# bikuta6/nbody-deep-sim

Measured on AMD Instinct MI355X. Metric: pair-interactions/sec, direct O(N^2) leapfrog N-body, fp32, higher is better.
Workload: dtype f32; 1 GPU; Plummer sphere, 65536 particles, direct all-pairs leapfrog step (BASELINE configs[1] shape: 65536 bodies per GPU); n_particles=65536, particles_per_gpu=65536, seed=1234, parallelism=single GPU

## Files before the change

nbody-deep-sim_amd/csrc/direct_force.hip:

```cpp
#include <hip/hip_runtime.h>
#include <string.h>
#include <stdint.h>

#include "../../include/nbd.h"
#include "direct_kernels.h"

namespace {

template <bool MASKED, int KU, bool UNI = false>
__global__ __launch_bounds__(64 * kWaves, KU == 4 ? 8 : 5) void accel_kernel(
    const f4* __restrict__ src, const SrcView sv, const f4* __restrict__ tgt,
    int n_tgt, int tgt_off, float eps2, float scale, float* __restrict__ out, int out_rows, int tile_len) {
  __shared__ f4 lds[kWaves * 2 * kChunk + kWaves * 6 * 64 / 4];
  {
    const int tz = blockIdx.z * tile_len;
    src += tz; tgt += tz; out += (size_t)tz * 3;
  }
  const int lane = threadIdx.x & 63;
  const int wave = __builtin_amdgcn_readfirstlane(threadIdx.x >> 6);
  const int t_base = blockIdx.x * kTgtPerWG;
  const int i0 = t_base + lane, i1 = t_base + 64 + lane;
  const f4 t0 = tgt[min(i0, n_tgt - 1)], t1 = tgt[min(i1, n_tgt - 1)];
  const f2 xi = {t0.x, t1.x}, yi = {t0.y, t1.y}, zi = {t0.z, t1.z};
  f2 ax = {0.f, 0.f}, ay = {0.f, 0.f}, az = {0.f, 0.f};
  f2 e2 = {eps2, eps2};
  asm volatile("" : "+v"(e2));

  const int jw = blockIdx.y * kWaves + wave;
  const int c_begin = jw * sv.cpw_q + min(jw, sv.cpw_r), c_end = c_begin + sv.cpw_q + (jw < sv.cpw_r ? 1 : 0);
  f4* stage = &lds[wave * 2 * kChunk];
  const f4* s_lane = src + lane;
  auto phys = [&](int c) { return c + (c >= sv.skip_c0 ? sv.skip_cn : 0); };
  if (c_begin < c_end)
    __builtin_amdgcn_global_load_lds(GPTR(s_lane + (size_t)phys(c_begin) * kChunk), LPTR(stage), 16, 0, 0);
  for (int c = c_begin; c < c_end; ++c) {
    const int b = (c - c_begin) & 1;
    if (c + 1 < c_end) {
      __builtin_amdgcn_global_load_lds(GPTR(s_lane + (size_t)phys(c + 1) * kChunk),
                                       LPTR(stage + (b ^ 1) * kChunk), 16, 0, 0);
      asm volatile("s_waitcnt vmcnt(1)" ::: "memory");
    } else {
      asm volatile("s_waitcnt vmcnt(0)" ::: "memory");
    }
    const f4* buf = stage + b * kChunk;
    const int pc = phys(c);
    const int j0 = pc * kChunk;
    if (MASKED || pc == sv.edge0 || pc == sv.edge1 || (UNI && pc == sv.tail)) {
#pragma unroll 4
      for (int j = 0; j < kChunk; ++j)
        interact<true, UNI>(buf[j], xi, yi, zi, e2, ax, ay, az, j0 + j, tgt_off + i0, tgt_off + i1, sv);
    } else {
#pragma unroll 1
      for (int j = 0; j < kChunk; j += KU) interact_block<KU, UNI>(buf + j, xi, yi, zi, e2, ax, ay, az);
    }
  }

  float* red = reinterpret_cast<float*>(&lds[kWaves * 2 * kChunk]);
  float* mine = red + wave * 6 * 64;
  mine[0 * 64 + lane] = ax.x; mine[1 * 64 + lane] = ax.y;
  mine[2 * 64 + lane] = ay.x; mine[3 * 64 + lane] = ay.y;
  mine[4 * 64 + lane] = az.x; mine[5 * 64 + lane] = az.y;
  __syncthreads();
  float* dst = out + ((size_t)blockIdx.y * out_rows + t_base) * 3;
  const int n_valid = min(kTgtPerWG, n_tgt - t_base) * 3;
  for (int o = threadIdx.x; o < n_valid; o += 64 * kWaves) {
    const int lt = o / 3, comp = o - lt * 3;
    const int idx = (comp * 2 + (lt >> 6)) * 64 + (lt & 63);
    float sum = red[idx];
#pragma unroll
    for (int w = 1; w < kWaves; ++w) sum += red[w * 6 * 64 + idx];
    dst[o] = __fmul_rn(scale, sum);
  }
}

constexpr int kSymTile = 1024;
constexpr int kSymChunks = kSymTile / kChunk;
constexpr int kSymSlots = 16;

__device__ __forceinline__ float rol1(float x) {
  return __int_as_float(__builtin_amdgcn_mov_dpp(__float_as_int(x), 0x134 , 0xf, 0xf, false));
}

__device__ __forceinline__ void sym_pair(const f4 p, const f2 xi, const f2 yi, const f2 zi, const f2 e2,
                                         f2& ax, f2& ay, f2& az, f2& rx, f2& ry, f2& rz) {
  const f2 dx = f2{p.x, p.x} - xi, dy = f2{p.y, p.y} - yi, dz = f2{p.z, p.z} - zi;
  f2 r2 = __builtin_elementwise_fma(dx, dx, e2);
  r2 = __builtin_elementwise_fma(dy, dy, r2);
  r2 = __builtin_elementwise_fma(dz, dz, r2);
  const f2 s = {__builtin_amdgcn_rsqf(r2.x), __builtin_amdgcn_rsqf(r2.y)};
  const f2 w = (s * s) * s;
  ax = __builtin_elementwise_fma(w, dx, ax);
  ay = __builtin_elementwise_fma(w, dy, ay);
  az = __builtin_elementwise_fma(w, dz, az);
  rx = __builtin_elementwise_fma(-w, dx, rx);
  ry = __builtin_elementwise_fma(-w, dy, ry);
  rz = __builtin_elementwise_fma(-w, dz, rz);
}

template <int SG>
__global__ __launch_bounds__(256 * SG, 2 * SG) void accel_sym_kernel(const f4* __restrict__ posm, int n, int m,
                                                                     int r0, int n_slots, float eps2,
                                                                     float* __restrict__ out) {
  constexpr int CPS = kSymChunks / SG;
  constexpr int kStageF4 = SG * 2 * 2 * kChunk;
  constexpr int kRedF = 2 * 4 * SG * 3 * 64;
  constexpr int kOwnF = SG * 4 * 12 * 64;
  constexpr int kLdsF = (kStageF4 * 4 + kRedF > kOwnF) ? kStageF4 * 4 + kRedF : kOwnF;
  __shared__ f4 lds[kLdsF / 4];
  float* const ldsf = reinterpret_cast<float*>(lds);

  const int half = m >> 1, mm = m - 1;
  const int rr = blockIdx.x / half, i = blockIdx.x - rr * half, r = r0 + rr;
  const int ta = i == 0 ? r % mm : (r + i) % mm;
  const int tb = i == 0 ? mm : (r - i + mm) % mm;
  const int slot = (r + 1) % n_slots;
  const bool init = r + 1 < n_slots;

  const int lane = threadIdx.x & 63;
  const int wave = __builtin_amdgcn_readfirstlane(threadIdx.x >> 6);
  const int tg = wave & 3, sg = wave >> 2;
  const int row0 = ta * kSymTile + tg * 256 + lane;
  const f4 q0 = posm[row0], q1 = posm[row0 + 64], q2 = posm[row0 + 128], q3 = posm[row0 + 192];
  const f2 xa = {q0.x, q1.x}, ya = {q0.y, q1.y}, za = {q0.z, q1.z};
  const f2 xb = {q2.x, q3.x}, yb = {q2.y, q3.y}, zb = {q2.z, q3.z};
  f2 axa = {0.f, 0.f}, aya = {0.f, 0.f}, aza = {0.f, 0.f}, axb = {0.f, 0.f}, ayb = {0.f, 0.f}, azb = {0.f, 0.f};
  f2 e2 = {eps2, eps2};
  asm volatile("" : "+v"(e2));

  f4* const stage = &lds[sg * 4 * kChunk];
  const int c0 = tb * kSymChunks + sg * CPS;
  const f4* const s_lane = posm + lane + (size_t)c0 * kChunk;
  auto fetch = [&](int c, int b) {
    __builtin_amdgcn_global_load_lds(GPTR(s_lane + c * kChunk), LPTR(stage + b * 2 * kChunk), 16, 0, 0);
    __builtin_amdgcn_global_load_lds(GPTR(s_lane + c * kChunk), LPTR(stage + b * 2 * kChunk + kChunk), 16, 0, 0);
  };
  if (tg == 3) {
    fetch(0, 0);
    asm volatile("s_waitcnt vmcnt(0)" ::: "memory");
  }
  __syncthreads();

  for (int c = 0; c < CPS; ++c) {
    const int b = c & 1;
    if (tg == 3 && c + 1 < CPS) fetch(c + 1, b ^ 1);
    float* const o_react = out + ((size_t)slot * n + (size_t)(c0 + c) * kChunk + lane) * 3 + tg;
    float old = 0.f;
    if (!init && tg < 3) old = *o_react;
    const f4* buf = stage + b * 2 * kChunk + lane;
    f2 rx = {0.f, 0.f}, ry = {0.f, 0.f}, rz = {0.f, 0.f};
#pragma unroll 2
    for (int k = 0; k < kChunk; ++k) {
      const f4 p = buf[k];
      sym_pair(p, xa, ya, za, e2, axa, aya, aza, rx, ry, rz);
      sym_pair(p, xb, yb, zb, e2, axb, ayb, azb, rx, ry, rz);
      rx = f2{rol1(rx.x), rol1(rx.y)};
      ry = f2{rol1(ry.x), rol1(ry.y)};
      rz = f2{rol1(rz.x), rol1(rz.y)};
    }
    float* const red = ldsf + kStageF4 * 4 + b * (4 * SG * 3 * 64);
    float* const mine = red + wave * 3 * 64;
    mine[lane] = rx.x + rx.y;
    mine[64 + lane] = ry.x + ry.y;
    mine[128 + lane] = rz.x + rz.y;
    if (tg == 3 && c + 1 < CPS) asm volatile("s_waitcnt vmcnt(0)" ::: "memory");
    __syncthreads();
    if (tg < 3) {
      const float* rs = red + (sg * 4) * 3 * 64 + tg * 64 + lane;
      const float v = ((rs[0] + rs[3 * 64]) + rs[6 * 64]) + rs[9 * 64];
      *o_react = init ? v : old + v;
    }
  }

  float* const o_own = out + ((size_t)slot * n + row0) * 3;
  const f2 own[6] = {axa, aya, aza, axb, ayb, azb};
  if (SG == 1) {
#pragma unroll
    for (int t = 0; t < 4; ++t)
#pragma unroll
      for (int comp = 0; comp < 3; ++comp) {
        const f2 v2 = own[(t >> 1) * 3 + comp];
        const float v = (t & 1) ? v2.y : v2.x;
        float* o = o_own + t * 64 * 3 + comp;
        *o = init ? v : *o + v;
      }
    return;
  }
  __syncthreads();
  float* const mo = ldsf + (sg * 4 + tg) * 12 * 64;
#pragma unroll
  for (int t = 0; t < 4; ++t)
#pragma unroll
    for (int comp = 0; comp < 3; ++comp) {
      const f2 v2 = own[(t >> 1) * 3 + comp];
      mo[(comp * 4 + t) * 64 + lane] = (t & 1) ? v2.y : v2.x;
    }
  __syncthreads();
  if (sg != 0) return;
#pragma unroll
  for (int t = 0; t < 4; ++t)
#pragma unroll
    for (int comp = 0; comp < 3; ++comp) {
      const float* src = ldsf + tg * 12 * 64 + (comp * 4 + t) * 64 + lane;
      float v = src[0];
#pragma unroll
      for (int g = 1; g < SG; ++g) v += src[g * 4 * 12 * 64];
      float* o = o_own + t * 64 * 3 + comp;
      *o = init ? v : *o + v;
    }
}

__global__ __launch_bounds__(256) void finish_kernel(const float* __restrict__ slabs, int n_slabs,
                                                     size_t slab_stride, float g, float* __restrict__ acc,
                                                     float* __restrict__ vel, float c_kick, int n3) {
  __shared__ float part[4][64];
  const int lane = threadIdx.x & 63, w = threadIdx.x >> 6;
  const int i = blockIdx.x * 64 + lane;
  float sum = 0.f;
  if (i < n3)
    for (int s = w; s < n_slabs; s += 4) sum += slabs[s * slab_stride + i];
  part[w][lane] = sum;
  __syncthreads();
  if (w != 0 || i >= n3) return;
  const float a = __fmul_rn(g, (part[0][lane] + part[1][lane]) + (part[2][lane] + part[3][lane]));
  acc[i] = a;
  if (vel) vel[i] = __fadd_rn(vel[i], __fmul_rn(c_kick, a));
}

__global__ __launch_bounds__(256) void pack_kernel(const float* __restrict__ pos,
                                                   const float* __restrict__ mass, int n, int n_pad,
                                                   f4* __restrict__ posm) {
  const int i = blockIdx.x * 256 + threadIdx.x;
  if (i >= n_pad) return;
  f4 v = {0.f, 0.f, 0.f, 0.f};
  if (i < n) v = f4{pos[3 * i], pos[3 * i + 1], pos[3 * i + 2], mass[i]};
  posm[i] = v;
}

__global__ __launch_bounds__(256) void kick_drift_kernel(float* __restrict__ pos, float* __restrict__ vel,
                                                         const float* __restrict__ acc,
                                                         const float* __restrict__ mass, int n, int n_pad,
                                                         float ck, float cd, f4* __restrict__ posm) {
  const int i = blockIdx.x * 256 + threadIdx.x;
  if (i >= n_pad) return;
  f4 pm = {0.f, 0.f, 0.f, 0.f};
  if (i < n) {
    float x[3];
#pragma unroll
    for (int k = 0; k < 3; ++k) {
      float v = vel[3 * i + k];
      if (acc) { v = __fadd_rn(v, __fmul_rn(ck, acc[3 * i + k])); vel[3 * i + k] = v; }
      x[k] = __fadd_rn(pos[3 * i + k], __fmul_rn(cd, v));
      pos[3 * i + k] = x[k];
    }
    pm = f4{x[0], x[1], x[2], mass ? mass[i] : 0.f};
  }
  if (posm) posm[i] = pm;
}

__global__ __launch_bounds__(256) void zero_f32_kernel(float* __restrict__ p, size_t n) {
  const size_t i = (size_t)blockIdx.x * 256 + threadIdx.x;
  if (i < n) p[i] = 0.f;
}

__global__ __launch_bounds__(256) void snapshot_kernel(const float* __restrict__ pos, const float* __restrict__ vel,
                                                       const float* __restrict__ acc, int n3, float* __restrict__ out) {
  const int i = blockIdx.x * 256 + threadIdx.x;
  if (i >= n3) return;
  out[i] = pos[i]; out[n3 + i] = vel[i]; out[2 * n3 + i] = acc[i];
}

__global__ __launch_bounds__(256) void axpy_kernel(float* __restrict__ y, const float* __restrict__ x,
                                                   float c, int n) {
  const int i = blockIdx.x * 256 + threadIdx.x;
  if (i < n) y[i] = __fadd_rn(y[i], __fmul_rn(c, x[i]));
}

__global__ __launch_bounds__(64 * kWaves) void energy_kernel(const f4* __restrict__ posm, int n, int n_chunks,
                                                             float soft_, int all_masked,
                                                             double* __restrict__ partial_u) {
  __shared__ f4 lds[kWaves * 2 * kChunk + 8];
  const int lane = threadIdx.x & 63;
  const int wave = __builtin_amdgcn_readfirstlane(threadIdx.x >> 6);
  const int t_base = blockIdx.x * kTgtPerWG;
  const int i0 = t_base + lane, i1 = t_base + 64 + lane;
  const f4 t0 = posm[min(i0, n - 1)], t1 = posm[min(i1, n - 1)];
  const f2 xi = {t0.x, t1.x}, yi = {t0.y, t1.y}, zi = {t0.z, t1.z};
  f2 u = {0.f, 0.f};
  f2 soft = {soft_, soft_};
  asm volatile("" : "+v"(soft));
  const int c_lo = t_base / kChunk;
  const int span = n_chunks - c_lo;
  const int parts = gridDim.y * kWaves;
  const int cpw = (span + parts - 1) / parts;
  const int jw = blockIdx.y * kWaves + wave;
  const int c_begin = min(c_lo + jw * cpw, n_chunks), c_end = min(c_begin + cpw, n_chunks);
  const int c_diag_end = (t_base + kTgtPerWG + kChunk - 1) / kChunk;
  f4* stage = &lds[wave * 2 * kChunk];
  const f4* s_lane = posm + lane;
  if (c_begin < c_end)
    __builtin_amdgcn_global_load_lds(GPTR(s_lane + (size_t)c_begin * kChunk), LPTR(stage), 16, 0, 0);
  for (int c = c_begin; c < c_end; ++c) {
    const int b = (c - c_begin) & 1;
    if (c + 1 < c_end) {
      __builtin_amdgcn_global_load_lds(GPTR(s_lane + (size_t)(c + 1) * kChunk), LPTR(stage + (b ^ 1) * kChunk), 16, 0, 0);
      asm volatile("s_waitcnt vmcnt(1)" ::: "memory");
    } else {
      asm volatile("s_waitcnt vmcnt(0)" ::: "memory");
    }
    const f4* buf = stage + b * kChunk;
    const int j0 = c * kChunk;
    if (all_masked || c < c_diag_end || c == n_chunks - 1) {
#pragma unroll 4
      for (int j = 0; j < kChunk; ++j) energy_pair<true>(buf[j], xi, yi, zi, soft, u, j0 + j, i0, i1, n);
    } else {
#pragma unroll 4
      for (int j = 0; j < kChunk; ++j) energy_pair<false>(buf[j], xi, yi, zi, soft, u, j0 + j, i0, i1, n);
    }
  }
  double acc = 0.0;
  if (i0 < n) acc += (double)t0.w * (double)u.x;
  if (i1 < n) acc += (double)t1.w * (double)u.y;
  for (int off = 32; off > 0; off >>= 1) acc += __shfl_down(acc, off);
  double* red = reinterpret_cast<double*>(&lds[kWaves * 2 * kChunk]);
  if (lane == 0) red[wave] = acc;
  __syncthreads();
  if (threadIdx.x == 0)
    partial_u[(size_t)blockIdx.y * gridDim.x + blockIdx.x] = (red[0] + red[1]) + (red[2] + red[3]);
}

__global__ __launch_bounds__(256) void kinetic_kernel(const f4* __restrict__ posm, const float* __restrict__ vel,
                                                      int n, double* __restrict__ partial_k) {
  __shared__ double red[4];
  const int i = blockIdx.x * 256 + threadIdx.x;
  double k = 0.0;
  if (i < n) {
    const float vx = vel[3 * i], vy = vel[3 * i + 1], vz = vel[3 * i + 2];
    const float v2 = __fadd_rn(__fadd_rn(__fmul_rn(vx, vx), __fmul_rn(vy, vy)), __fmul_rn(vz, vz));
    k = (double)__fmul_rn(__fmul_rn(0.5f, posm[i].w), v2);
  }
  for (int off = 32; off > 0; off >>= 1) k += __shfl_down(k, off);
  if ((threadIdx.x & 63) == 0) red[threadIdx.x >> 6] = k;
  __syncthreads();
  if (threadIdx.x == 0) partial_k[blockIdx.x] = (red[0] + red[1]) + (red[2] + red[3]);
}

__global__ __launch_bounds__(256) void energy_final_kernel(const double* __restrict__ pu, int nu,
                                                           const double* __restrict__ pk, int nk, float g,
                                                           double* __restrict__ out) {
  __shared__ double ru[4], rk[4];
  double u = 0.0, k = 0.0;
  for (int b = threadIdx.x; b < nu; b += 256) u += pu[b];
  for (int b = threadIdx.x; b < nk; b += 256) k += pk[b];
  for (int off = 32; off > 0; off >>= 1) { u += __shfl_down(u, off); k += __shfl_down(k, off); }
  if ((threadIdx.x & 63) == 0) { ru[threadIdx.x >> 6] = u; rk[threadIdx.x >> 6] = k; }
  __syncthreads();
  if (threadIdx.x == 0) {
    out[0] = -(double)g * ((ru[0] + ru[1]) + (ru[2] + ru[3]));
    out[1] = (rk[0] + rk[1]) + (rk[2] + rk[3]);
  }
}

inline int energy_slabs(int groups) {
  int s = (4096 + groups - 1) / groups;
  return s < 1 ? 1 : (s > 32 ? 32 : s);
}

struct AccelPlan { int groups, slabs, n_chunks, cpw, variant; };

constexpr int kCUs = 256;
double plan_cost(int groups, int n_chunks, int slabs) {
  static const double eff[6] = {1.0, 0.70, 0.935, 0.975, 0.99, 1.0};
  const int waves = slabs * kWaves, q = n_chunks / waves, r = n_chunks % waves;
  const int wgs = groups * slabs, per_cu = ceil_div(wgs, kCUs);
  const int heavy_per_cu = ceil_div(groups * ceil_div(r, kWaves), kCUs);
  const double chunks = (double)per_cu * q + (heavy_per_cu < per_cu ? heavy_per_cu : per_cu);
  return chunks / eff[per_cu < 5 ? per_cu : 5] * (per_cu <= 5 ? 1.03 : 1.0) + 0.25 * per_cu;
}

AccelPlan plan_chunks(int n_chunks, int n_tgt) {
  AccelPlan p;
  p.variant = 0;
  p.groups = ceil_div(n_tgt, kTgtPerWG);
  p.n_chunks = n_chunks;
  int cap = n_chunks / kWaves;
  cap = cap < 1 ? 1 : (cap > kMaxSlabs ? kMaxSlabs : cap);
  int slabs;
  const int pref = ceil_div(8192, p.groups), cap_pref = n_chunks / (16 * kWaves);
  if ((pref < cap_pref ? pref : cap_pref) * p.groups >= 10 * kCUs) {
    slabs = pref < cap_pref ? pref : cap_pref;
    const int min_slabs = ceil_div(n_chunks, kWaves * 64);
    if (slabs < min_slabs) slabs = min_slabs;
  } else {
    slabs = 1;
    double best = plan_cost(p.groups, n_chunks, 1);
    for (int s = 2; s <= cap; ++s) {
      const double c = plan_cost(p.groups, n_chunks, s);
      if (c < best * 0.999) { best = c; slabs = s; }
    }
  }
  if (slabs > kMaxSlabs) slabs = kMaxSlabs;
  if (slabs < 1) slabs = 1;
  p.slabs = slabs;
  p.cpw = ceil_div(n_chunks, p.slabs * kWaves);
  return p;
}

AccelPlan plan_accel(int n_src, int n_tgt) { return plan_chunks(ceil_div(n_src, kChunk), n_tgt); }

inline int check(hipError_t e) { return e == hipSuccess ? 0 : (int)e; }
inline int launch_status() { return check(hipGetLastError()); }

SrcView full_view(int n_src, const AccelPlan& p) {
  SrcView v;
  v.n_src = n_src; v.n_chunks = p.n_chunks; v.cpw_q = 0; v.cpw_r = 0;
  v.skip_c0 = p.n_chunks; v.skip_cn = 0; v.ex_lo = 0; v.ex_hi = 0; v.edge0 = -1; v.edge1 = -1;
  v.tail = (n_src % kChunk) ? n_src / kChunk : -1;
  return v;
}

int excluded_view(int n_src, int ex_lo, int ex_hi, SrcView* v) {
  const int phys = ceil_div(n_src, kChunk);
  int c0 = ceil_div(ex_lo, kChunk), c1 = ex_hi / kChunk;
  if (ex_hi >= n_src) c1 = phys;
  if (c1 < c0) c1 = c0;
  if (v) {
    v->n_src = n_src; v->skip_c0 = c0; v->skip_cn = c1 - c0; v->ex_lo = ex_lo; v->ex_hi = ex_hi;
    v->edge0 = (ex_lo % kChunk) ? ex_lo / kChunk : -1;
    v->edge1 = (ex_hi % kChunk && ex_hi < n_src) ? ex_hi / kChunk : -1;
    if (ex_hi <= ex_lo) { v->skip_c0 = phys; v->skip_cn = 0; v->edge0 = v->edge1 = -1; }
    v->tail = (n_src % kChunk) ? n_src / kChunk : -1;
  }
  return ex_hi <= ex_lo ? phys : phys - (c1 - c0);
}

int launch_accel(const float* posm_src, SrcView sv, const float* posm_tgt, int n_tgt, int off,
                 float eps2, float direct_scale, float* slabs_or_acc, const AccelPlan& p,
                 hipStream_t st, bool uniform = false, int out_rows = 0, int tiles = 1, int tile_len = 0) {
  dim3 grid(p.groups, p.slabs, tiles), block(64 * kWaves);
  if (out_rows <= 0) out_rows = n_tgt;
  const f4* s = reinterpret_cast<const f4*>(posm_src);
  const f4* t = reinterpret_cast<const f4*>(posm_tgt);
  sv.n_chunks = p.n_chunks;
  sv.cpw_q = p.n_chunks / (p.slabs * kWaves); sv.cpw_r = p.n_chunks % (p.slabs * kWaves);
  const bool masked = eps2 < kEps2Masked;
#define NBD_LAUNCH(M, K, U) accel_kernel<M, K, U><<<grid, block, 0, st>>>(s, sv, t, n_tgt, off, eps2, direct_scale, slabs_or_acc, out_rows, tile_len)
  if (uniform) {
    if (p.variant == 1) { if (masked) NBD_LAUNCH(true, 4, true); else NBD_LAUNCH(false, 4, true); }
    else                { if (masked) NBD_LAUNCH(true, 8, true); else NBD_LAUNCH(false, 8, true); }
  } else {
    if (p.variant == 1) { if (masked) NBD_LAUNCH(true, 4, false); else NBD_LAUNCH(false, 4, false); }
    else                { if (masked) NBD_LAUNCH(true, 8, false); else NBD_LAUNCH(false, 8, false); }
  }
#undef NBD_LAUNCH
  return launch_status();
}

bool misaligned16(const void* p) { return (reinterpret_cast<uintptr_t>(p) & 15) != 0; }

struct SymPlan { int m, core, rem, slots, total_slots; };

SymPlan plan_sym(int n) {
  SymPlan p;
  p.m = n / kSymTile;
  p.m &= ~1;
  p.core = p.m * kSymTile;
  p.rem = n - p.core;
  p.slots = p.m < kSymSlots ? p.m : kSymSlots;
  p.total_slots = p.slots + (p.rem > 0 ? 1 : 0);
  return p;
}

size_t sym_workspace_bytes(int n) {
  const SymPlan p = plan_sym(n);
  return p.m < 2 ? 0 : (size_t)p.total_slots * n * 3 * sizeof(float);
}

constexpr int kSymStepMinN = 65536;
bool sym_step(int n, float eps2) { return n >= kSymStepMinN && eps2 >= kEps2Masked; }

int launch_sym(const float* posm, int n, float eps2, float* slots, hipStream_t st, int variant = 0) {
  const SymPlan sp = plan_sym(n);
  const f4* pm = reinterpret_cast<const f4*>(posm);
  AccelPlan dp;
  dp.groups = kSymTile / kTgtPerWG; dp.slabs = 1; dp.n_chunks = kSymChunks; dp.variant = 0;
  dp.cpw = ceil_div(kSymChunks, kWaves);
  int rc = launch_accel(posm, full_view(kSymTile, dp), posm, kSymTile, 0, eps2, 1.0f, slots, dp, st, true, n, sp.m,
                        kSymTile);
  if (rc) return rc;
  const int rounds = sp.m - 1;
  for (int r0 = 0; r0 < rounds;) {
    const int r1 = r0 == 0 ? (sp.slots - 1 < rounds ? sp.slots - 1 : rounds) : (r0 + sp.slots < rounds ? r0 + sp.slots : rounds);
    const int wgs = (r1 - r0) * (sp.m / 2);
    if (variant == 1) accel_sym_kernel<2><<<wgs, 512, 0, st>>>(pm, n, sp.m, r0, sp.slots, eps2, slots);
    else accel_sym_kernel<4><<<wgs, 1024, 0, st>>>(pm, n, sp.m, r0, sp.slots, eps2, slots);
    if ((rc = launch_status())) return rc;
    r0 = r1;
  }
  if (sp.rem == 0) return 0;
  AccelPlan tp;
  tp.groups = ceil_div(sp.rem, kTgtPerWG); tp.slabs = sp.total_slots; tp.n_chunks = ceil_div(n, kChunk); tp.variant = 0;
  tp.cpw = ceil_div(tp.n_chunks, tp.slabs * kWaves);
  rc = launch_accel(posm, full_view(n, tp), posm + (size_t)sp.core * 4, sp.rem, sp.core, eps2, 1.0f,
                    slots + (size_t)sp.core * 3, tp, st, true, n);
  if (rc) return rc;
  SrcView sv;
  AccelPlan cp;
  cp.n_chunks = excluded_view(n, 0, sp.core, &sv);
  cp.groups = sp.core / kTgtPerWG; cp.slabs = 1; cp.variant = 0; cp.cpw = ceil_div(cp.n_chunks, kWaves);
  return launch_accel(posm, sv, posm, sp.core, 0, eps2, 1.0f, slots + (size_t)sp.slots * n * 3, cp, st, true, n);
}


}

extern "C" {

int nbd_abi_version(void) { return NBD_ABI_VERSION; }

size_t nbd_struct_size(const char* name) {
  if (!name) return 0;
#define NBD_SZ(T) if (!strcmp(name, #T)) return sizeof(T);
  NBD_SZ(nbd_gnn_layer_args) NBD_SZ(nbd_gnn_forward_args) NBD_SZ(nbd_knn_pq_args) NBD_SZ(nbd_gnn_train_args)
  NBD_SZ(nbd_gnn_train_grads) NBD_SZ(nbd_cc_train_args) NBD_SZ(nbd_cc_train_grads) NBD_SZ(nbd_cc_pairs_job)
#undef NBD_SZ
  return 0;
}

const char* nbd_strerror(int code) {
  if (code == 0) return "ok";
  if (code == NBD_E_BADARG) return "nbd: bad argument (null/negative/misaligned)";
  if (code == NBD_E_WORKSPACE) return "nbd: workspace too small";
  if (code == NBD_E_UNSUPPORTED) return "nbd: unsupported configuration";
  if (code > 0) return hipGetErrorString((hipError_t)code);
  return "nbd: unknown error";
}

int nbd_posm_padded_len(int n) { return n <= 0 ? 0 : ceil_div(n, kChunk) * kChunk; }

int nbd_pack_posm_f32(const float* pos, const float* mass, int n, float* posm, nbd_stream_t stream) {
  if (n < 0 || (n > 0 && (!pos || !mass || !posm)) || misaligned16(posm)) return NBD_E_BADARG;
  if (n == 0) return 0;
  const int n_pad = nbd_posm_padded_len(n);
  pack_kernel<<<ceil_div(n_pad, 256), 256, 0, (hipStream_t)stream>>>(pos, mass, n, n_pad,
                                                                    reinterpret_cast<f4*>(posm));
  return launch_status();
}

size_t nbd_accel_workspace_bytes(int n_src, int n_tgt) {
  if (n_src <= 0 || n_tgt <= 0) return 0;
  const AccelPlan p = plan_accel(n_src, n_tgt);
  return p.slabs > 1 ? (size_t)p.slabs * n_tgt * 3 * sizeof(float) : 0;
}

int nbd_accel_plan(int n_src, int n_tgt, int* groups, int* slabs, int* chunks_per_wave) {
  if (n_src <= 0 || n_tgt <= 0) return NBD_E_BADARG;
  const AccelPlan p = plan_accel(n_src, n_tgt);
  if (groups) *groups = p.groups;
  if (slabs) *slabs = p.slabs;
  if (chunks_per_wave) *chunks_per_wave = p.cpw;
  return 0;
}

size_t nbd_step_workspace_bytes(int n) {
  if (n <= 0) return 0;
  const size_t all_pairs = (size_t)plan_accel(n, n).slabs * n * 3 * sizeof(float);
  const size_t sym = sym_step(n, kEps2Masked) ? sym_workspace_bytes(n) : 0;
  return sym > all_pairs ? sym : all_pairs;
}

size_t nbd_accel_sym_workspace_bytes(int n) { return n <= 0 ? 0 : sym_workspace_bytes(n); }

int nbd_accel_sym_uniform_f32(const float* posm, int n, float softening_sq, float g_const, float mass_value,
                              float* acc_out, void* workspace, size_t workspace_bytes, int variant, nbd_stream_t stream) {
  if (n < 0 || (n > 0 && (!posm || !acc_out)) || misaligned16(posm) || variant < 0 || variant > 1) return NBD_E_BADARG;
  if (n == 0) return 0;
  if (plan_sym(n).m < 2 || softening_sq < kEps2Masked) return NBD_E_UNSUPPORTED;
  if (!workspace || workspace_bytes < sym_workspace_bytes(n)) return NBD_E_WORKSPACE;
  hipStream_t st = (hipStream_t)stream;
  float* slots = static_cast<float*>(workspace);
  int rc = launch_sym(posm, n, softening_sq, slots, st, variant);
  if (rc) return rc;
  const int n3 = 3 * n;
  finish_kernel<<<ceil_div(n3, 64), 256, 0, st>>>(slots, plan_sym(n).total_slots, (size_t)n3, g_const * mass_value,
                                                   acc_out, nullptr, 0.f, n3);
  return launch_status();
}

int nbd_accel_f32(const float* posm_src, int n_src, const float* posm_tgt, int n_tgt,
                  int tgt_global_offset, float softening_sq, float g_const, float* acc_out,
                  void* workspace, size_t workspace_bytes, nbd_stream_t stream) {
  if (n_src < 0 || n_tgt < 0) return NBD_E_BADARG;
  if (n_tgt == 0) return 0;
  if (!acc_out || !posm_tgt || misaligned16(posm_tgt)) return NBD_E_BADARG;
  hipStream_t st = (hipStream_t)stream;
  if (n_src == 0) {
    zero_f32_kernel<<<ceil_div(n_tgt * 3, 256), 256, 0, st>>>(acc_out, (size_t)n_tgt * 3);
    return launch_status();
  }
  if (!posm_src || misaligned16(posm_src)) return NBD_E_BADARG;
  const AccelPlan p = plan_accel(n_src, n_tgt);
  if (p.slabs == 1)
    return launch_accel(posm_src, full_view(n_src, p), posm_tgt, n_tgt, tgt_global_offset, softening_sq,
                        g_const, acc_out, p, st);
  const size_t need = (size_t)p.slabs * n_tgt * 3 * sizeof(float);
  if (!workspace || workspace_bytes < need) return NBD_E_WORKSPACE;
  float* slabs = static_cast<float*>(workspace);
  int rc = launch_accel(posm_src, full_view(n_src, p), posm_tgt, n_tgt, tgt_global_offset, softening_sq,
                        1.0f, slabs, p, st);
  if (rc) return rc;
  const int n3 = n_tgt * 3;
  finish_kernel<<<ceil_div(n3, 64), 256, 0, st>>>(slabs, p.slabs, (size_t)n3, g_const, acc_out,
                                                   nullptr, 0.f, n3);
  return launch_status();
}

size_t nbd_accel_tuned_workspace_bytes(int n_tgt, int slabs) {
  if (n_tgt <= 0 || slabs <= 0) return 0;
  return (size_t)slabs * n_tgt * 3 * sizeof(float);
}

int nbd_accel_tuned_f32(const float* posm_src, int n_src, int exclude_lo, int exclude_hi, const float* posm_tgt,
                        int n_tgt, int tgt_global_offset, float softening_sq, float g_const, float* acc_out,
                        void* workspace, size_t workspace_bytes, int slabs, int variant, nbd_stream_t stream) {
  if (n_src <= 0 || n_tgt <= 0 || slabs < 1 || slabs > kMaxSlabs || variant < 0 || variant > 1) return NBD_E_BADARG;
  if (exclude_lo < 0 || exclude_hi < exclude_lo || exclude_hi > n_src) return NBD_E_BADARG;
  if (!acc_out || !posm_tgt || !posm_src || misaligned16(posm_tgt) || misaligned16(posm_src)) return NBD_E_BADARG;
  if (!workspace || workspace_bytes < nbd_accel_tuned_workspace_bytes(n_tgt, slabs)) return NBD_E_WORKSPACE;
  hipStream_t st = (hipStream_t)stream;
  SrcView sv;
  AccelPlan p;
  p.n_chunks = excluded_view(n_src, exclude_lo, exclude_hi, &sv);
  p.groups = ceil_div(n_tgt, kTgtPerWG);
  p.slabs = slabs;
  p.variant = variant;
  p.cpw = ceil_div(p.n_chunks > 0 ? p.n_chunks : 1, slabs * kWaves);
  float* sl = static_cast<float*>(workspace);
  const int n3 = n_tgt * 3;
  if (p.n_chunks == 0) {
    zero_f32_kernel<<<ceil_div(n3, 256), 256, 0, st>>>(acc_out, (size_t)n3);
    return launch_status();
  }
  int rc = launch_accel(posm_src, sv, posm_tgt, n_tgt, tgt_global_offset, softening_sq, 1.0f, sl, p, st);
  if (rc) return rc;
  finish_kernel<<<ceil_div(n3, 64), 256, 0, st>>>(sl, p.slabs, (size_t)n3, g_const, acc_out, nullptr, 0.f, n3);
  return launch_status();
}

struct ShardPlan { AccelPlan local, remote; };

ShardPlan plan_shard_uncached(int n_total, int lo, int n_local) {
  ShardPlan sp;
  sp.local = plan_chunks(ceil_div(n_local, kChunk), n_local);
  const int rc = excluded_view(n_total, lo, lo + n_local, nullptr);
  sp.remote = plan_chunks(rc > 0 ? rc : 1, n_local);
  if (rc == 0) { sp.remote.slabs = 0; sp.remote.n_chunks = 0; }
  return sp;
}

ShardPlan plan_shard(int n_total, int lo, int n_local) {
  struct Memo { int n_total, lo, n_local; ShardPlan sp; };
  thread_local Memo memo[4] = {{-1, 0, 0, {}}, {-1, 0, 0, {}}, {-1, 0, 0, {}}, {-1, 0, 0, {}}};
  thread_local int next = 0;
  for (const Memo& m : memo)
    if (m.n_total == n_total && m.lo == lo && m.n_local == n_local) return m.sp;
  Memo& m = memo[next];
  next = (next + 1) & 3;
  m.n_total = n_total; m.lo = lo; m.n_local = n_local;
  m.sp = plan_shard_uncached(n_total, lo, n_local);
  return m.sp;
}

int nbd_shard_plan(int n_total, int lo, int n_local, int* slabs_local, int* cpw_local, int* slabs_remote,
                   int* cpw_remote) {
  if (n_total <= 0 || lo < 0 || n_local <= 0 || lo + n_local > n_total) return NBD_E_BADARG;
  const ShardPlan sp = plan_shard(n_total, lo, n_local);
  if (slabs_local) *slabs_local = sp.local.slabs;
  if (cpw_local) *cpw_local = sp.local.cpw;
  if (slabs_remote) *slabs_remote = sp.remote.slabs;
  if (cpw_remote) *cpw_remote = sp.remote.cpw;
  return 0;
}

size_t nbd_shard_workspace_bytes(int n_total, int lo, int n_local) {
  if (n_total <= 0 || lo < 0 || n_local <= 0 || lo + n_local > n_total) return 0;
  const ShardPlan sp = plan_shard(n_total, lo, n_local);
  return (size_t)(sp.local.slabs + sp.remote.slabs) * n_local * 3 * sizeof(float);
}

int nbd_shard_force_local_f32(const float* posm_local, int n_local, float softening_sq, void* workspace,
                              size_t workspace_bytes, int n_total, int lo, nbd_stream_t stream) {
  if (n_local < 0 || n_total < 0 || lo < 0 || lo + n_local > n_total) return NBD_E_BADARG;
  if (n_local == 0) return 0;
  if (!posm_local || misaligned16(posm_local)) return NBD_E_BADARG;
  if (!workspace || workspace_bytes < nbd_shard_workspace_bytes(n_total, lo, n_local)) return NBD_E_WORKSPACE;
  const ShardPlan sp = plan_shard(n_total, lo, n_local);
  return launch_accel(posm_local, full_view(n_local, sp.local), posm_local, n_local, 0, softening_sq, 1.0f,
                      static_cast<float*>(workspace), sp.local, (hipStream_t)stream);
}

int nbd_shard_force_remote_f32(const float* posm_all, int n_total, const float* posm_local, int n_local, int lo,
                               float softening_sq, float g_const, float* acc_out, float* vel, float c_kick,
                               void* workspace, size_t workspace_bytes, nbd_stream_t stream) {
  if (n_local < 0 || n_total < 0 || lo < 0 || lo + n_local > n_total) return NBD_E_BADARG;
  if (n_local == 0) return 0;
  if (!posm_all || !posm_local || !acc_out || misaligned16(posm_all) || misaligned16(posm_local)) return NBD_E_BADARG;
  if (!workspace || workspace_bytes < nbd_shard_workspace_bytes(n_total, lo, n_local)) return NBD_E_WORKSPACE;
  hipStream_t st = (hipStream_t)stream;
  const ShardPlan sp = plan_shard(n_total, lo, n_local);
  float* slabs = static_cast<float*>(workspace);
  const int n3 = 3 * n_local;
  if (sp.remote.slabs > 0) {
    SrcView sv;
    excluded_view(n_total, lo, lo + n_local, &sv);
    int rc = launch_accel(posm_all, sv, posm_local, n_local, lo, softening_sq, 1.0f,
                          slabs + (size_t)sp.local.slabs * n3, sp.remote, st);
    if (rc) return rc;
  }
  finish_kernel<<<ceil_div(n3, 64), 256, 0, st>>>(slabs, sp.local.slabs + sp.remote.slabs, (size_t)n3, g_const,
                                                   acc_out, vel, c_kick, n3);
  return launch_status();
}

int nbd_shard_force_local_uniform_f32(const float* posm_local, int n_local, float softening_sq, void* workspace,
                                      size_t workspace_bytes, int n_total, int lo, nbd_stream_t stream) {
  if (n_local < 0 || n_total < 0 || lo < 0 || lo + n_local > n_total) return NBD_E_BADARG;
  if (n_local == 0) return 0;
  if (!posm_local || misaligned16(posm_local)) return NBD_E_BADARG;
  if (!workspace || workspace_bytes < nbd_shard_workspace_bytes(n_total, lo, n_local)) return NBD_E_WORKSPACE;
  const ShardPlan sp = plan_shard(n_total, lo, n_local);
  return launch_accel(posm_local, full_view(n_local, sp.local), posm_local, n_local, 0, softening_sq, 1.0f,
                      static_cast<float*>(workspace), sp.local, (hipStream_t)stream, true);
}

int nbd_shard_force_remote_uniform_f32(const float* posm_all, int n_total, const float* posm_local, int n_local, int lo,
                                       float softening_sq, float g_const, float mass_value, float* acc_out, float* vel,
                                       float c_kick, void* workspace, size_t workspace_bytes, nbd_stream_t stream) {
  if (n_local < 0 || n_total < 0 || lo < 0 || lo + n_local > n_total) return NBD_E_BADARG;
  if (n_local == 0) return 0;
  if (!posm_all || !posm_local || !acc_out || misaligned16(posm_all) || misaligned16(posm_local)) return NBD_E_BADARG;
  if (!workspace || workspace_bytes < nbd_shard_workspace_bytes(n_total, lo, n_local)) return NBD_E_WORKSPACE;
  hipStream_t st = (hipStream_t)stream;
  const ShardPlan sp = plan_shard(n_total, lo, n_local);
  float* slabs = static_cast<float*>(workspace);
  const int n3 = 3 * n_local;
  if (sp.remote.slabs > 0) {
    SrcView sv;
    excluded_view(n_total, lo, lo + n_local, &sv);
    int rc = launch_accel(posm_all, sv, posm_local, n_local, lo, softening_sq, 1.0f,
                          slabs + (size_t)sp.local.slabs * n3, sp.remote, st, true);
    if (rc) return rc;
  }
  finish_kernel<<<ceil_div(n3, 64), 256, 0, st>>>(slabs, sp.local.slabs + sp.remote.slabs, (size_t)n3, g_const * mass_value,
                                                   acc_out, vel, c_kick, n3);
  return launch_status();
}

int nbd_kick_drift_f32(float* pos, float* vel, const float* acc, const float* mass, int n,
                       float c_kick, float c_drift, float* posm, nbd_stream_t stream) {
  if (n < 0 || (n > 0 && (!pos || !vel)) || (posm && (!mass || misaligned16(posm)))) return NBD_E_BADARG;
  if (n == 0) return 0;
  const int n_pad = posm ? nbd_posm_padded_len(n) : n;
  kick_drift_kernel<<<ceil_div(n_pad, 256), 256, 0, (hipStream_t)stream>>>(
      pos, vel, acc, mass, n, n_pad, c_kick, c_drift, reinterpret_cast<f4*>(posm));
  return launch_status();
}

int nbd_kick_f32(float* vel, const float* acc, int n, float c, nbd_stream_t stream) {
  if (n < 0 || (n > 0 && (!vel || !acc))) return NBD_E_BADARG;
  if (n == 0) return 0;
  axpy_kernel<<<ceil_div(3 * n, 256), 256, 0, (hipStream_t)stream>>>(vel, acc, c, 3 * n);
  return launch_status();
}

int nbd_drift_f32(float* pos, const float* vel, int n, float c, nbd_stream_t stream) {
  if (n < 0 || (n > 0 && (!pos || !vel))) return NBD_E_BADARG;
  if (n == 0) return 0;
  axpy_kernel<<<ceil_div(3 * n, 256), 256, 0, (hipStream_t)stream>>>(pos, vel, c, 3 * n);
  return launch_status();
}

int nbd_snapshot_f32(const float* pos, const float* vel, const float* acc, int n, float* out, nbd_stream_t stream) {
  if (n < 0 || (n > 0 && (!pos || !vel || !acc || !out))) return NBD_E_BADARG;
  if (n == 0) return 0;
  snapshot_kernel<<<ceil_div(3 * n, 256), 256, 0, (hipStream_t)stream>>>(pos, vel, acc, 3 * n, out);
  return launch_status();
}

int nbd_leapfrog_step_ev_f32(float* pos, float* vel, const float* acc_in, float* acc_out,
                          const float* mass, int n, float dt_half, float dt, float softening_sq,
                          float g_const, float* posm, void* workspace, size_t workspace_bytes,
                          nbd_stream_t stream, void* ev_force_begin, void* ev_force_end) {
  if (n < 0) return NBD_E_BADARG;
  if (n == 0) return 0;
  if (!pos || !vel || !acc_in || !acc_out || !mass || !posm || misaligned16(posm)) return NBD_E_BADARG;
  hipStream_t st = (hipStream_t)stream;
  const AccelPlan p = plan_accel(n, n);
  const size_t need = (size_t)p.slabs * n * 3 * sizeof(float);
  if (!workspace || workspace_bytes < need) return NBD_E_WORKSPACE;
  int rc = nbd_kick_drift_f32(pos, vel, acc_in, mass, n, dt_half, dt, posm, stream);
  if (rc) return rc;
  float* slabs = static_cast<float*>(workspace);
  if (ev_force_begin && (rc = check(hipEventRecord((hipEvent_t)ev_force_begin, st)))) return rc;
  rc = launch_accel(posm, full_view(n, p), posm, n, 0, softening_sq, 1.0f, slabs, p, st);
  if (rc) return rc;
  if (ev_force_end && (rc = check(hipEventRecord((hipEvent_t)ev_force_end, st)))) return rc;
  const int n3 = 3 * n;
  finish_kernel<<<ceil_div(n3, 64), 256, 0, st>>>(slabs, p.slabs, (size_t)n3, g_const, acc_out, vel,
                                                   dt_half, n3);
  return launch_status();
}

int nbd_leapfrog_step_uniform_f32(float* pos, float* vel, const float* acc_in, float* acc_out, const float* mass,
                                  float mass_value, int n, float dt_half, float dt, float softening_sq, float g_const,
                                  float* posm, void* workspace, size_t workspace_bytes, nbd_stream_t stream,
                                  void* ev_force_begin, void* ev_force_end) {
  if (n < 0) return NBD_E_BADARG;
  if (n == 0) return 0;
  if (!pos || !vel || !acc_in || !acc_out || !mass || !posm || misaligned16(posm)) return NBD_E_BADARG;
  hipStream_t st = (hipStream_t)stream;
  const bool sym = sym_step(n, softening_sq);
  const AccelPlan p = plan_accel(n, n);
  const size_t need = sym ? sym_workspace_bytes(n) : (size_t)p.slabs * n * 3 * sizeof(float);
  if (!workspace || workspace_bytes < need) return NBD_E_WORKSPACE;
  int rc = nbd_kick_drift_f32(pos, vel, acc_in, mass, n, dt_half, dt, posm, stream);
  if (rc) return rc;
  float* slabs = static_cast<float*>(workspace);
  if (ev_force_begin && (rc = check(hipEventRecord((hipEvent_t)ev_force_begin, st)))) return rc;
  if (sym) rc = launch_sym(posm, n, softening_sq, slabs, st);
  else rc = launch_accel(posm, full_view(n, p), posm, n, 0, softening_sq, 1.0f, slabs, p, st, true);
  if (rc) return rc;
  if (ev_force_end && (rc = check(hipEventRecord((hipEvent_t)ev_force_end, st)))) return rc;
  const int n3 = 3 * n;
  const int n_slabs = sym ? plan_sym(n).total_slots : p.slabs;
  finish_kernel<<<ceil_div(n3, 64), 256, 0, st>>>(slabs, n_slabs, (size_t)n3, g_const * mass_value, acc_out, vel,
                                                   dt_half, n3);
  return launch_status();
}

int nbd_leapfrog_step_f32(float* pos, float* vel, const float* acc_in, float* acc_out,
                          const float* mass, int n, float dt_half, float dt, float softening_sq,
                          float g_const, float* posm, void* workspace, size_t workspace_bytes,
                          nbd_stream_t stream) {
  return nbd_leapfrog_step_ev_f32(pos, vel, acc_in, acc_out, mass, n, dt_half, dt, softening_sq, g_const,
                                  posm, workspace, workspace_bytes, stream, nullptr, nullptr);
}

int nbd_euler_step_f32(float* pos, float* vel, float* acc_out, const float* mass, int n, float dt,
                       float softening_sq, float g_const, float* posm, void* workspace,
                       size_t workspace_bytes, nbd_stream_t stream) {
  if (n < 0) return NBD_E_BADARG;
  if (n == 0) return 0;
  if (!pos || !vel || !acc_out || !mass || !posm || misaligned16(posm)) return NBD_E_BADARG;
  hipStream_t st = (hipStream_t)stream;
  const AccelPlan p = plan_accel(n, n);
  const size_t need = (size_t)p.slabs * n * 3 * sizeof(float);
  if (!workspace || workspace_bytes < need) return NBD_E_WORKSPACE;
  int rc = nbd_pack_posm_f32(pos, mass, n, posm, stream);
  if (rc) return rc;
  float* slabs = static_cast<float*>(workspace);
  rc = launch_accel(posm, full_view(n, p), posm, n, 0, softening_sq, 1.0f, slabs, p, st);
  if (rc) return rc;
  const int n3 = 3 * n;
  finish_kernel<<<ceil_div(n3, 64), 256, 0, st>>>(slabs, p.slabs, (size_t)n3, g_const, acc_out, vel, dt, n3);
  rc = launch_status();
  if (rc) return rc;
  return nbd_drift_f32(pos, vel, n, dt, stream);
}

size_t nbd_energy_workspace_bytes(int n) {
  if (n <= 0) return 0;
  const int groups = ceil_div(n, kTgtPerWG);
  return ((size_t)groups * energy_slabs(groups) + (size_t)ceil_div(n, 256)) * sizeof(double);
}

int nbd_energy_f32(const float* posm, const float* vel, int n, float softening, float g_const,
                   double* out_uk, void* workspace, size_t workspace_bytes, nbd_stream_t stream) {
  if (n < 0 || !out_uk) return NBD_E_BADARG;
  hipStream_t st = (hipStream_t)stream;
  if (n == 0) {
    zero_f32_kernel<<<1, 256, 0, st>>>(reinterpret_cast<float*>(out_uk), 4);
    return launch_status();
  }
  if (!posm || !vel || misaligned16(posm)) return NBD_E_BADARG;
  if (!workspace || workspace_bytes < nbd_energy_workspace_bytes(n)) return NBD_E_WORKSPACE;
  const int groups = ceil_div(n, kTgtPerWG), slabs = energy_slabs(groups), nk = ceil_div(n, 256);
  double* pu = static_cast<double*>(workspace);
  double* pk = pu + (size_t)groups * slabs;
  const f4* pm = reinterpret_cast<const f4*>(posm);
  energy_kernel<<<dim3(groups, slabs), 64 * kWaves, 0, st>>>(pm, n, ceil_div(n, kChunk), softening,
                                                           softening > 0.f ? 0 : 1, pu);
  int rc = launch_status();
  if (rc) return rc;
  kinetic_kernel<<<nk, 256, 0, st>>>(pm, vel, n, pk);
  rc = launch_status();
  if (rc) return rc;
  energy_final_kernel<<<1, 256, 0, st>>>(pu, groups * slabs, pk, nk, g_const, out_uk);
  return launch_status();
}

}
```

Before: 5963 billion pair-interactions/s.

## Add register-tiled symmetric pair kernel with LDS-resident source tile and lane-rotated reactions

Adds a new symmetric tile-pair kernel that loads the whole source tile once into LDS (xy/z split layout, duplicated for rotation) and gives each thread 8 target bodies in registers. Reaction forces are accumulated per lane and rotated across the wave each step, with explicit scheduling barriers to interleave independent rsqrt chains. The uniform leapfrog step now uses this variant by default. It raises register pressure and occupancy is bounded at 512 threads x 4, and the reduction layout becomes more intricate.

```diff
diff --git a/nbody-deep-sim_amd/csrc/direct_force.hip b/nbody-deep-sim_amd/csrc/direct_force.hip
--- a/nbody-deep-sim_amd/csrc/direct_force.hip
+++ b/nbody-deep-sim_amd/csrc/direct_force.hip
@@ -97,6 +97,16 @@
   rz = __builtin_elementwise_fma(-w, dz, rz);
 }
 
+__device__ __forceinline__ void sym_round_match(int wg, int m, int r0, int n_slots, int& ta, int& tb, int& slot,
+                                                bool& init) {
+  const int half = m >> 1, mm = m - 1;
+  const int rr = wg / half, i = wg - rr * half, r = r0 + rr;
+  ta = i == 0 ? r % mm : (r + i) % mm;
+  tb = i == 0 ? mm : (r - i + mm) % mm;
+  slot = (r + 1) % n_slots;
+  init = r + 1 < n_slots;
+}
+
 template <int SG>
 __global__ __launch_bounds__(256 * SG, 2 * SG) void accel_sym_kernel(const f4* __restrict__ posm, int n, int m,
                                                                      int r0, int n_slots, float eps2,
@@ -109,12 +119,9 @@
   __shared__ f4 lds[kLdsF / 4];
   float* const ldsf = reinterpret_cast<float*>(lds);
 
-  const int half = m >> 1, mm = m - 1;
-  const int rr = blockIdx.x / half, i = blockIdx.x - rr * half, r = r0 + rr;
-  const int ta = i == 0 ? r % mm : (r + i) % mm;
-  const int tb = i == 0 ? mm : (r - i + mm) % mm;
-  const int slot = (r + 1) % n_slots;
-  const bool init = r + 1 < n_slots;
+  int ta, tb, slot;
+  bool init;
+  sym_round_match(blockIdx.x, m, r0, n_slots, ta, tb, slot, init);
 
   const int lane = threadIdx.x & 63;
   const int wave = __builtin_amdgcn_readfirstlane(threadIdx.x >> 6);
@@ -207,6 +214,144 @@
       float* o = o_own + t * 64 * 3 + comp;
       *o = init ? v : *o + v;
     }
+}
+
+constexpr int kSym2Pairs = kSymChunks / 2;
+constexpr int kSym2T = 8;
+constexpr int kSym2G = 2;
+
+__global__ __launch_bounds__(512, 4) void accel_sym2_kernel(const f4* __restrict__ posm, int n, int m, int r0,
+                                                            int n_slots, float eps2, float* __restrict__ out) {
+  constexpr int kXyF = kSym2Pairs * 128 * 4;
+  constexpr int kZF = kSym2Pairs * 128 * 2;
+  constexpr int kReactF = 2 * 8 * 6 * 64;
+  constexpr int kOwnF = 8 * 3 * kSym2T * 64;
+  static_assert(kXyF + kZF + kReactF == kOwnF, "one 48-KiB LDS image");
+  __shared__ f4 lds[kOwnF / 4];
+  float* const ldsf = reinterpret_cast<float*>(lds);
+  f4* const xy = lds;
+  f2* const zz = reinterpret_cast<f2*>(ldsf + kXyF);
+  float* const react = ldsf + kXyF + kZF;
+
+  int ta, tb, slot;
+  bool init;
+  sym_round_match(blockIdx.x, m, r0, n_slots, ta, tb, slot, init);
+
+  const int lane = threadIdx.x & 63;
+  const int wave = __builtin_amdgcn_readfirstlane(threadIdx.x >> 6);
+  const int tg = wave & 1, sg = wave >> 1;
+  {
+    const f4 u = posm[tb * kSymTile + wave * kChunk + lane];
+    const f4 v = posm[tb * kSymTile + (wave + kSym2Pairs) * kChunk + lane];
+    const f4 q = {u.x, v.x, u.y, v.y};
+    const f2 z = {u.z, v.z};
+    xy[wave * 128 + lane] = q; xy[wave * 128 + 64 + lane] = q;
+    zz[wave * 128 + lane] = z; zz[wave * 128 + 64 + lane] = z;
+  }
+  const int row0 = ta * kSymTile + tg * 512 + lane;
+  f2 txy[kSym2T], tzz[kSym2T / 2];
+  f2 ax[kSym2T], ay[kSym2T], az[kSym2T];
+#pragma unroll
+  for (int t = 0; t < kSym2T; ++t) {
+    const f4 q = posm[row0 + t * 64];
+    txy[t] = f2{q.x, q.y};
+    if (t & 1) tzz[t >> 1].y = q.z; else tzz[t >> 1].x = q.z;
+    ax[t] = ay[t] = az[t] = f2{0.f, 0.f};
+  }
+  f2 e2 = {eps2, eps2};
+  asm volatile("" : "+v"(e2));
+  __syncthreads();
+
+#pragma unroll 1
+  for (int j = 0; j < 2; ++j) {
+    const int p = sg * 2 + j;
+    const f4* const bxy = xy + p * 128 + lane;
+    const f2* const bz = zz + p * 128 + lane;
+    f2 rx = {0.f, 0.f}, ry = {0.f, 0.f}, rz = {0.f, 0.f};
+#pragma unroll 1
+    for (int k = 0; k < kChunk; ++k) {
+      const f4 a = bxy[k];
+      const f2 sx = {a.x, a.y}, sy = {a.z, a.w}, sz = bz[k];
+#pragma unroll
+      for (int t = 0; t < kSym2T; ++t) asm volatile("" : "+v"(txy[t]));
+#pragma unroll
+      for (int t = 0; t < kSym2T / 2; ++t) asm volatile("" : "+v"(tzz[t]));
+#pragma unroll
+      for (int g = 0; g < kSym2T; g += kSym2G) {
+        f2 dx[kSym2G], dy[kSym2G], dz[kSym2G], s[kSym2G], w[kSym2G];
+#pragma unroll
+        for (int u = 0; u < kSym2G; ++u) {
+          const int t = g + u;
+          const float tz = (t & 1) ? tzz[t >> 1].y : tzz[t >> 1].x;
+          dx[u] = sx - f2{txy[t].x, txy[t].x}; dy[u] = sy - f2{txy[t].y, txy[t].y}; dz[u] = sz - f2{tz, tz};
+        }
+        __builtin_amdgcn_sched_barrier(0);
+#pragma unroll
+        for (int u = 0; u < kSym2G; ++u) s[u] = __builtin_elementwise_fma(dx[u], dx[u], e2);
+        __builtin_amdgcn_sched_barrier(0);
+#pragma unroll
+        for (int u = 0; u < kSym2G; ++u) s[u] = __builtin_elementwise_fma(dy[u], dy[u], s[u]);
+        __builtin_amdgcn_sched_barrier(0);
+#pragma unroll
+        for (int u = 0; u < kSym2G; ++u) s[u] = __builtin_elementwise_fma(dz[u], dz[u], s[u]);
+        __builtin_amdgcn_sched_barrier(0);
+#pragma unroll
+        for (int u = 0; u < kSym2G; ++u) s[u] = f2{__builtin_amdgcn_rsqf(s[u].x), __builtin_amdgcn_rsqf(s[u].y)};
+        __builtin_amdgcn_sched_barrier(0);
+#pragma unroll
+        for (int u = 0; u < kSym2G; ++u) w[u] = s[u] * s[u];
+        __builtin_amdgcn_sched_barrier(0);
+#pragma unroll
+        for (int u = 0; u < kSym2G; ++u) w[u] = w[u] * s[u];
+        __builtin_amdgcn_sched_barrier(0);
+#pragma unroll
+        for (int u = 0; u < kSym2G; ++u) {
+          const int t = g + u;
+          ax[t] = __builtin_elementwise_fma(w[u], dx[u], ax[t]);
+          ay[t] = __builtin_elementwise_fma(w[u], dy[u], ay[t]);
+          az[t] = __builtin_elementwise_fma(w[u], dz[u], az[t]);
+          rx = __builtin_elementwise_fma(-w[u], dx[u], rx);
+          ry = __builtin_elementwise_fma(-w[u], dy[u], ry);
+          rz = __builtin_elementwise_fma(-w[u], dz[u], rz);
+        }
+      }
+      rx = f2{rol1(rx.x), rol1(rx.y)};
+      ry = f2{rol1(ry.x), rol1(ry.y)};
+      rz = f2{rol1(rz.x), rol1(rz.y)};
+    }
+    float* const mine = react + (j * 8 + wave) * 6 * 64 + lane;
+    mine[0 * 64] = rx.x; mine[1 * 64] = rx.y;
+    mine[2 * 64] = ry.x; mine[3 * 64] = ry.y;
+    mine[4 * 64] = rz.x; mine[5 * 64] = rz.y;
+  }
+  __syncthreads();
+
+  float* const o_b = out + ((size_t)slot * n + (size_t)tb * kSymTile) * 3;
+  for (int o = threadIdx.x; o < kSymTile * 3; o += 512) {
+    const int row = o / 3, comp = o - row * 3;
+    const int c = row >> 6, l = row & 63, p = c & (kSym2Pairs - 1), hf = c / kSym2Pairs;
+    const float* rs = react + ((p & 1) * 8 + (p >> 1) * 2) * 6 * 64 + (comp * 2 + hf) * 64 + l;
+    const float v = rs[0] + rs[6 * 64];
+    o_b[o] = init ? v : o_b[o] + v;
+  }
+  __syncthreads();
+#pragma unroll
+  for (int t = 0; t < kSym2T; ++t) {
+    float* const mo = ldsf + ((sg * 2 + tg) * 3 * kSym2T + t) * 64 + lane;
+    mo[0 * kSym2T * 64] = ax[t].x + ax[t].y;
+    mo[1 * kSym2T * 64] = ay[t].x + ay[t].y;
+    mo[2 * kSym2T * 64] = az[t].x + az[t].y;
+  }
+  __syncthreads();
+  float* const o_a = out + ((size_t)slot * n + (size_t)ta * kSymTile) * 3;
+  for (int o = threadIdx.x; o < kSymTile * 3; o += 512) {
+    const int row = o / 3, comp = o - row * 3;
+    const int g = row >> 9, t = (row >> 6) & (kSym2T - 1), l = row & 63;
+    const float* os = ldsf + ((g * 3 + comp) * kSym2T + t) * 64 + l;
+    constexpr int kSg = 2 * 3 * kSym2T * 64;
+    const float v = ((os[0] + os[kSg]) + os[2 * kSg]) + os[3 * kSg];
+    o_a[o] = init ? v : o_a[o] + v;
+  }
 }
 
 __global__ __launch_bounds__(256) void finish_kernel(const float* __restrict__ slabs, int n_slabs,
@@ -491,7 +636,8 @@
   for (int r0 = 0; r0 < rounds;) {
     const int r1 = r0 == 0 ? (sp.slots - 1 < rounds ? sp.slots - 1 : rounds) : (r0 + sp.slots < rounds ? r0 + sp.slots : rounds);
     const int wgs = (r1 - r0) * (sp.m / 2);
-    if (variant == 1) accel_sym_kernel<2><<<wgs, 512, 0, st>>>(pm, n, sp.m, r0, sp.slots, eps2, slots);
+    if (variant == 2) accel_sym2_kernel<<<wgs, 512, 0, st>>>(pm, n, sp.m, r0, sp.slots, eps2, slots);
+    else if (variant == 1) accel_sym_kernel<2><<<wgs, 512, 0, st>>>(pm, n, sp.m, r0, sp.slots, eps2, slots);
     else accel_sym_kernel<4><<<wgs, 1024, 0, st>>>(pm, n, sp.m, r0, sp.slots, eps2, slots);
     if ((rc = launch_status())) return rc;
     r0 = r1;
@@ -572,7 +718,7 @@
 
 int nbd_accel_sym_uniform_f32(const float* posm, int n, float softening_sq, float g_const, float mass_value,
                               float* acc_out, void* workspace, size_t workspace_bytes, int variant, nbd_stream_t stream) {
-  if (n < 0 || (n > 0 && (!posm || !acc_out)) || misaligned16(posm) || variant < 0 || variant > 1) return NBD_E_BADARG;
+  if (n < 0 || (n > 0 && (!posm || !acc_out)) || misaligned16(posm) || variant < 0 || variant > 2) return NBD_E_BADARG;
   if (n == 0) return 0;
   if (plan_sym(n).m < 2 || softening_sq < kEps2Masked) return NBD_E_UNSUPPORTED;
   if (!workspace || workspace_bytes < sym_workspace_bytes(n)) return NBD_E_WORKSPACE;
@@ -826,7 +972,7 @@
   if (rc) return rc;
   float* slabs = static_cast<float*>(workspace);
   if (ev_force_begin && (rc = check(hipEventRecord((hipEvent_t)ev_force_begin, st)))) return rc;
-  if (sym) rc = launch_sym(posm, n, softening_sq, slabs, st);
+  if (sym) rc = launch_sym(posm, n, softening_sq, slabs, st, 2);
   else rc = launch_accel(posm, full_view(n, p), posm, n, 0, softening_sq, 1.0f, slabs, p, st, true);
   if (rc) return rc;
   if (ev_force_end && (rc = check(hipEventRecord((hipEvent_t)ev_force_end, st)))) return rc;
```

Result: faster. 6508 billion pair-interactions/s (median of 6 runs) (+9.1%).
